# Structural-Variant-Calling-with-Pepper/pepper-thesis

Measured on AMD Instinct MI355X. Metric: pileup windows/sec (whole node) + Mbp/sec inferred, HG003 chr20 ONT R9, higher is better.
Workload: dtype f32

## Files before the change

### pepper_thesis_amd/csrc/rnn_bf16.hpp

```cpp
#pragma once
#include "pv_common.hpp"
#include "rnn_plan.hpp"

struct pv_gemm_desc {
    const unsigned char* A;
    const unsigned char* W;
    const float* bias;
    float* C;
    int64_t M;
    int N, K, splits, quads;
    const char* prof_name;
    int terms;
};
int pv_gemm_bf16x3_async(pv_ctx* ctx, const pv_gemm_desc& g, hipStream_t st);
int pv_gemm_bf16x3_prepare();
int pv_upload_split8(const float* w, size_t N, size_t K, unsigned char** d_split, std::vector<void*>& owned);
int pv_upload_split3(const float* w, size_t N, size_t K, unsigned char** d_planes, std::vector<void*>& owned);

struct pv_rec_desc {
    int cell;
    int enc;
    const float* G;
    const unsigned char* wp;
    const unsigned char* wx;
    const float* bias;
    const float* bias_hn;
    const void* x;
    int64_t x_row_bytes;
    int x_t0, xf, x_signed;
    int64_t B, Bp;
    int T;
    const float* h0;
    float* h_out;
    float* out_f32;
    unsigned char* out_tm;
    unsigned char* out_bm;
    int mt;
    const char* prof_name;
    int tr16;
    const unsigned char* dense_w;
    float* dense_part;
    int x6;
};
int pv_rec_bf16_async(pv_ctx* ctx, const pv_rec_desc& d, hipStream_t st);
int pv_rec_bf16_prepare();
int pv_pack_rec_bf16(const pv_rnn_dir* dirs, int cell, int kx, unsigned char** d_wp, unsigned char** d_wx, std::vector<void*>& owned,
                     int pieces = 2);
int pv_pack_gru16_bf16(const pv_rnn_dir* dirs, int kx, unsigned char** d_wp, unsigned char** d_wx, std::vector<void*>& owned);

struct pv_tail_desc {
    const float* part;
    int splits;
    int64_t part_rows;
    const float* b1;
    const unsigned char* wp;
    const float* b[4];
    const float* wo;
    const float* bo;
    float* probs;
    int64_t B;
    unsigned* epoch;
    const int* err;
};
int pv_tail_bf16_async(pv_ctx* ctx, const pv_tail_desc& d, hipStream_t st);
int pv_tail_bf16_prepare();
int pv_pack_tail_bf16(const float* const* w, unsigned char** d_wp, std::vector<void*>& owned);

struct pv_p2_bf16_weights {
    unsigned char* enc_wp = nullptr;
    unsigned char* enc_wx = nullptr;
    unsigned char* dec_wp = nullptr;
    float* enc_bias = nullptr;
    float* enc_bias_hn = nullptr;
    float* dec_bias_hn = nullptr;
    unsigned char* dec_wih_s = nullptr;
    unsigned char* dense_frag = nullptr;
    unsigned char* dense_frag16 = nullptr;
    unsigned char* enc16_wp = nullptr;
    unsigned char* enc16_wx = nullptr;
    unsigned char* dec16_wp = nullptr;
// ... 9 lines not shown
```

### pepper_thesis_amd/csrc/rnn_p1.hip

```cpp
#include "pv_common.hpp"
#include "rnn_bf16.hpp"
#include "rnn_f32.hpp"
#include "rnn_pack_host.hpp"

#include <algorithm>
#include <optional>

namespace {

constexpr int T_STEPS = PV_P1_T;
constexpr int F_IN = PV_P1_F;
constexpr int H = PV_P1_H;
constexpr int ROWS = PV_P1_ROWS;
constexpr int HEAD_N = PV_HEAD_N;
constexpr int HEAD_K = PV_HEAD_K;
constexpr int HEAD_MAX_SPLITS = PV_HEAD_MAX_SPLITS;

}

struct pv_rnn_p1 {
    float* enc_wp[2] = {nullptr, nullptr};
    float* dec_wp[2] = {nullptr, nullptr};
    float* enc_bias = nullptr; float* dec_bias = nullptr;
    float* enc_wps[2] = {nullptr, nullptr};
// ... 52 lines not shown
        pack_lstm(w->encoder, F_IN, 32, f ? 16 : 32, wp, bias);
        if ((rc = pv_dev_upload(wp, &m->enc_wp[f], m->owned))) return rc;
        if (!f && (rc = pv_dev_upload(bias, &m->enc_bias, m->owned))) return rc;
        pack_lstm(w->decoder, 2 * H, 2 * H, f ? 16 : 32, wp, bias);
        if ((rc = pv_dev_upload(wp, &m->dec_wp[f], m->owned))) return rc;
        if (!f && (rc = pv_dev_upload(bias, &m->dec_bias, m->owned))) return rc;
    }
    for (int f = 0; f < 2; f++) {
        pack_lstm_split(w->encoder, F_IN, 32, f ? 2 : 4, wp);
        if ((rc = pv_dev_upload(wp, &m->enc_wps[f], m->owned))) return rc;
        pack_lstm_split(w->decoder, 2 * H, 2 * H, f ? 2 : 4, wp);
        if ((rc = pv_dev_upload(wp, &m->dec_wps[f], m->owned))) return rc;
    }
    if ((rc = pv_dev_zeros(PV_LSTM_HX_BYTES, &m->sp_hx, m->owned)) || (rc = pv_dev_zeros(PV_LSTM_FLAGS_BYTES, &m->sp_flags, m->owned)) ||
        (rc = pv_dev_zeros(64, &m->sp_err, m->owned)) || (rc = pv_dev_zeros(64, &m->sp_epoch, m->owned)))
        return rc;
    pack_linear(w->linear_w[0], HEAD_K, 32, wp);
    if ((rc = pv_dev_upload(wp, &m->w1p, m->owned)) || (rc = pv_dev_upload(w->linear_b[0], HEAD_N, &m->b1, m->owned))) return rc;
    for (int i = 0; i < 4; i++) {
        for (int f = 0; f < 2; f++) {
            pack_linear(w->linear_w[i + 1], HEAD_N, f ? 16 : 32, wp);
            if ((rc = pv_dev_upload(wp, &m->wlp[f][i], m->owned))) return rc;
        }
        if ((rc = pv_dev_upload(w->linear_b[i + 1], HEAD_N, &m->bl[i], m->owned))) return rc;
    }
    if ((rc = pv_dev_upload(w->out_w, 3 * HEAD_N, &m->wo, m->owned)) || (rc = pv_dev_upload(w->out_b, 3, &m->bo, m->owned))) return rc;
    std::vector<float> wcat((size_t)2048 * 512), bcat(2048);
    for (int d = 0; d < 2; d++) {
        memcpy(&wcat[(size_t)d * 1024 * 512], w->decoder[d].w_ih, (size_t)1024 * 512 * sizeof(float));
        for (int n = 0; n < 1024; n++) bcat[d * 1024 + n] = w->decoder[d].b_ih[n] + w->decoder[d].b_hh[n];
    }
    if ((rc = pv_dev_upload(bcat, &m->dec_bias_cat, m->owned))) return rc;
    if (dtype == PV_DTYPE_F32) {
        if ((rc = pv_pack_rec_bf16(w->encoder, 4, F_IN, &m->enc_r6, nullptr, m->owned, 3))) return rc;
        if ((rc = pv_pack_rec_bf16(w->decoder, 4, 0, &m->dec_r6, nullptr, m->owned, 3))) return rc;
        if ((rc = pv_upload_split3(wcat.data(), 2048, 512, &m->dec_wih_p3, m->owned))) return rc;
        if ((rc = pv_upload_split3(w->linear_w[0], HEAD_N, HEAD_K, &m->w1_p3, m->owned))) return rc;
        if ((rc = pv_gemm_bf16x3_prepare()) || (rc = pv_rec_bf16_prepare())) return rc;
    }
    if (dtype == PV_DTYPE_BF16_INPUT_GEMM) {
        if ((rc = pv_upload_split8(wcat.data(), 2048, 512, &m->dec_wih_s, m->owned))) return rc;
        if ((rc = pv_upload_split8(w->linear_w[0], HEAD_N, HEAD_K, &m->w1_s, m->owned))) return rc;
        if ((rc = pv_pack_rec_bf16(w->encoder, 4, F_IN, &m->enc_rb, nullptr, m->owned))) return rc;
        if ((rc = pv_pack_rec_bf16(w->decoder, 4, 0, &m->dec_rb, nullptr, m->owned))) return rc;
        const float* tail_w[4] = {w->linear_w[1], w->linear_w[2], w->linear_w[3], w->linear_w[4]};
        if ((rc = pv_pack_tail_bf16(tail_w, &m->tail_wb, m->owned))) return rc;
        if ((rc = pv_gemm_bf16x3_prepare()) || (rc = pv_rec_bf16_prepare()) || (rc = pv_tail_bf16_prepare())) return rc;
    }
    if ((rc = pv_lstm_f32_prepare()) || (rc = pv_head_f32_prepare())) return rc;
    return PV_OK;
}

static int launch_tail(pv_ctx* ctx, const pv_p1_plan& pl, const float* part, int64_t part_rows, float* d_probs, int64_t B, hipStream_t st) {
    const pv_rnn_p1* m = ctx->p1;
    pv_head_tail_desc t = {};
    t.rows = pl.tail_rows; t.part = part; t.b1 = m->b1; t.splits = pl.splits; t.part_rows = part_rows;
    t.wo = m->wo; t.bo = m->bo; t.probs = d_probs; t.B = B; t.epoch = m->sp_epoch; t.err = m->sp_err;
    for (int i = 0; i < 4; i++) { t.wp[i] = m->wlp[pl.tail_rows == 16 ? 1 : 0][i]; t.b[i] = m->bl[i]; }
    int rc = pv_head_tail_async(ctx, t, st);
    if (rc) return rc;
    PV_HIP(hipGetLastError());
    return PV_OK;
}

struct P1Chain {
    int terms;
    const unsigned char *enc_rec, *dec_rec;
    const void *dec_wih, *w1;
// ... 166 lines not shown
```

### pepper_thesis_amd/csrc/rnn_pack_host.hpp

```cpp
#pragma once
#include <cstddef>
#include <cstdint>
#include <vector>

#include "../../include/pepper_hip.h"
#include "split3_host.hpp"

constexpr int PV_PACK_LSTM_H = 256;
constexpr int PV_PACK_GRU_H = 128;
constexpr int PV_PACK_NCLS = 5;
constexpr int PV_PACK_HEAD_N = 512;

static inline float pack_wval(const pv_rnn_dir& dir, int K, int KP, int HID, int n, int k) {
    if (k < KP) return k < K ? dir.w_ih[(size_t)n * K + k] : 0.0f;
    return dir.w_hh[(size_t)n * HID + (k - KP)];
}

static inline void pack_put_pieces(uint16_t* slot, int lane, int j, float v, int pieces = 2) {
    uint16_t p[3];
    split3_bits(v, p);
    for (int q = 0; q < pieces; q++) slot[512 * q + lane * 8 + j] = p[q];
}

static inline void split8_rows(const float* w, size_t N, size_t K, std::vector<uint16_t>& out) {
// ... 129 lines not shown

static inline void pack_rec_bf16(const pv_rnn_dir* dirs, int cell, int kx, int pieces, std::vector<uint16_t>& wp, std::vector<uint16_t>& wx) {
    const int NG = cell, HID = cell == 4 ? PV_PACK_LSTM_H : PV_PACK_GRU_H, NW = HID / 32, KS_H = HID / 16;
    const int KS_X = kx ? (cell == 4 ? 2 : 1) : 0;
    const bool xres = kx && cell == 3;
    const int nslot = (xres ? 0 : KS_X * NG) + KS_H * NG;
    const size_t SL = (size_t)pieces * 512;
    wp.assign((size_t)2 * NW * nslot * SL, 0);
    wx.assign(xres ? (size_t)2 * NW * NG * 1024 : 0, 0);
    for (int d = 0; d < 2; d++)
        for (int w = 0; w < NW; w++) {
            auto fill = [&](uint16_t* dst, bool xpart, int ks, int g) {
                for (int lane = 0; lane < 64; lane++)
                    for (int j = 0; j < 8; j++) {
                        const int n = g * HID + 32 * w + (lane & 31), k = 16 * ks + 8 * (lane >> 5) + j;
                        float v;
                        if (xpart) v = k < kx ? dirs[d].w_ih[(size_t)n * kx + k] : 0.0f;
                        else v = dirs[d].w_hh[(size_t)n * HID + k];
                        pack_put_pieces(dst, lane, j, v, pieces);
                    }
            };
            uint16_t* base = wp.data() + (size_t)(d * NW + w) * nslot * SL;
            int slot = 0;
            if (!xres)
                for (int ks = 0; ks < KS_X; ks++)
                    for (int g = 0; g < NG; g++) fill(base + (size_t)(slot++) * SL, true, ks, g);
            for (int ks = 0; ks < KS_H; ks++)
                for (int g = 0; g < NG; g++) fill(base + (size_t)(slot++) * SL, false, ks, g);
            if (xres)
                for (int g = 0; g < NG; g++) fill(wx.data() + ((size_t)(d * NW + w) * NG + g) * 1024, true, 0, g);
        }
}

static inline void pack_gru16_bf16(const pv_rnn_dir* dirs, int kx, std::vector<uint16_t>& wp, std::vector<uint16_t>& wx) {
    const int HID = PV_PACK_GRU_H, NW = 4;
    wp.assign((size_t)2 * NW * 24 * 1024, 0);
    wx.assign(kx ? (size_t)2 * NW * 6 * 1024 : 0, 0);
    for (int d = 0; d < 2; d++)
        for (int w = 0; w < NW; w++)
            for (int g = 0; g < 3; g++)
                for (int nt = 0; nt < 2; nt++) {
                    auto fill = [&](uint16_t* dst, bool xpart, int ks) {
                        for (int lane = 0; lane < 64; lane++)
                            for (int j = 0; j < 8; j++) {
                                const int n = g * HID + 32 * w + 16 * nt + (lane & 15), k = 32 * ks + 8 * (lane >> 4) + j;
                                const float v = xpart ? (k < kx ? dirs[d].w_ih[(size_t)n * kx + k] : 0.0f) : dirs[d].w_hh[(size_t)n * HID + k];
                                pack_put_pieces(dst, lane, j, v);
                            }
                    };
                    for (int ks = 0; ks < 4; ks++) fill(wp.data() + ((size_t)(d * NW + w) * 24 + (ks * 3 + g) * 2 + nt) * 1024, false, ks);
                    if (kx) fill(wx.data() + ((size_t)(d * NW + w) * 6 + g * 2 + nt) * 1024, true, 0);
                }
}

static inline void pack_tail_bf16(const float* const* w, std::vector<uint16_t>& wp) {
    constexpr int N = PV_PACK_HEAD_N, KS = N / 16;
    wp.assign((size_t)8 * 4 * KS * 2 * 1024, 0);
    for (int wv = 0; wv < 8; wv++)
        for (int l = 0; l < 4; l++)
            for (int ks = 0; ks < KS; ks++)
                for (int g = 0; g < 2; g++) {
                    uint16_t* dst = wp.data() + ((((size_t)wv * 4 + l) * KS + ks) * 2 + g) * 1024;
                    for (int lane = 0; lane < 64; lane++)
                        for (int j = 0; j < 8; j++) {
                            const int n = 64 * wv + 32 * g + (lane & 31), k = 16 * ks + 8 * (lane >> 5) + j;
                            pack_put_pieces(dst, lane, j, w[l][(size_t)n * N + k]);
// ... 32 lines not shown
```

### pepper_thesis_amd/csrc/rnn_rec_bf16.hip

```cpp
#include "rnn_bf16.hpp"
#include "mfma_tiles.hpp"
#include "rnn_math.hpp"
#include "rnn_p2_head.hpp"
#include "rnn_pack_host.hpp"

#include <algorithm>
#include <type_traits>
#include <cstdlib>

namespace {

using namespace pvdev;
typedef __bf16 bf16x8 __attribute__((ext_vector_type(8)));
typedef __bf16 bf16x4 __attribute__((ext_vector_type(4)));

__device__ __forceinline__ void split3_rest(float h, __bf16& x1, __bf16& x2) {
#pragma clang fp contract(off)
    const float r1 = h - (float)(__bf16)h;
    x1 = (__bf16)r1;
    x2 = (__bf16)(r1 - (float)x1);
}
__device__ __forceinline__ unsigned split8_off(unsigned k) { return (k >> 3) * 32u + (k & 7u) * 2u; }

template <int NG, bool ENC, int MT = 1, bool X6 = false> struct RecCfg {
    static constexpr int HID = NG == 4 ? 256 : 128;
    static constexpr int NW = HID / 32, NTHR = 64 * NW;
    static constexpr int KS_H = HID / 16;
    static constexpr int XK = ENC ? (NG == 4 ? 32 : 16) : 0;
    static constexpr int KS_X = XK / 16;
    static constexpr bool XRES = ENC && NG == 3;
    static constexpr bool WRES = NG == 3 && !(ENC && MT == 2);
    static constexpr int NSLOT = (XRES ? 0 : KS_X * NG) + KS_H * NG;
    static constexpr int D = ((NG == 3 && ENC) || (NG == 4 && MT == 2) || X6) ? 4 : 8;
    static constexpr int NA = NG + ((NG == 3 && ENC) ? 1 : 0);
    static constexpr int HS = HID * (X6 ? 8 : 4) + 16;
    static constexpr int H12 = X6 ? HID * 4 : 0;
    static constexpr int XS = XK * 2 + 16;
    static_assert(NSLOT % D == 0, "ring depth must divide the stream length");
};

struct RecArgs {
    const float* G;
    const unsigned char* wp;
    const unsigned char* wx;
    const float* bias;
    const float* bias_hn;
    const unsigned char* x;
    int64_t x_row_bytes;
    int x_t0, xf, x_signed;
    int64_t B, Bp;
    int T;
    const float* h0;
    float* h_out;
    float* out_f32;
    unsigned char* out_tm;
    unsigned char* out_bm;
    int n_tiles;
    const unsigned char* dw;
    float* dpart;
};

template <int NG, int MT, int NA, int D, int NTOT, int I0, int NKS, bool XP, bool X6 = false, int H12 = 0, typename Hook>
__device__ __forceinline__ void ring_bf16(f32x16 (&acc)[MT][NA], const unsigned char* __restrict__ At, int m_stride,
                                          __amdgpu_buffer_rsrc_t wr, f32x4 (&bq)[D][X6 ? 3 : 2], unsigned lane16, Hook&& hook) {
    constexpr int KSB = XP ? 32 : 64;
    constexpr int NP = X6 ? 3 : 2, SB = NP * 1024;
    bf16x8 ap[X6 && !XP ? 3 : 2][MT];
#pragma unroll
    for (int i = 0; i < NKS * NG; i++) {
        {
// ... 13 lines not shown
#pragma unroll
                    for (int j = 0; j < 8; j++) ap[0][m][j] = (__bf16)(j < 4 ? lo[j] : hi[j - 4]);
                } else {
                    ap[0][m] = *reinterpret_cast<const bf16x8*>(At + m * m_stride + ks * KSB);
                    if (!XP) ap[1][m] = *reinterpret_cast<const bf16x8*>(At + m * m_stride + ks * KSB + 16);
                }
            }
        }
        __builtin_amdgcn_sched_barrier(0);
        {
            const int ai = (XP && NG == 3 && g == 2) ? 3 : g;
            const int rs = (I0 + i) % D;
            const bf16x8 bh = __builtin_bit_cast(bf16x8, bq[rs][0]), bl = __builtin_bit_cast(bf16x8, bq[rs][1]);
#pragma unroll
            for (int m = 0; m < MT; m++) {
                if constexpr (X6) {
                    const bf16x8 b2 = __builtin_bit_cast(bf16x8, bq[rs][2]);
                    if constexpr (!XP) {
                        acc[m][ai] = __builtin_amdgcn_mfma_f32_32x32x16_bf16(ap[2][m], bh, acc[m][ai], 0, 0, 0);
                        acc[m][ai] = __builtin_amdgcn_mfma_f32_32x32x16_bf16(ap[1][m], bl, acc[m][ai], 0, 0, 0);
                    }
                    acc[m][ai] = __builtin_amdgcn_mfma_f32_32x32x16_bf16(ap[0][m], b2, acc[m][ai], 0, 0, 0);
                }
                acc[m][ai] = __builtin_amdgcn_mfma_f32_32x32x16_bf16(ap[0][m], bh, acc[m][ai], 0, 0, 0);
                acc[m][ai] = __builtin_amdgcn_mfma_f32_32x32x16_bf16(ap[0][m], bl, acc[m][ai], 0, 0, 0);
                if (!XP) acc[m][ai] = __builtin_amdgcn_mfma_f32_32x32x16_bf16(ap[1][m], bh, acc[m][ai], 0, 0, 0);
            }
        }
        hook(i);
        __builtin_amdgcn_sched_barrier(0);
    }
}

#ifndef PV_REC_ABL
#define PV_REC_ABL 0
#endif
#ifdef PV_REC_STAMPS
__device__ unsigned long long g_rec_stamps[8];
#define RSTAMP(i) { unsigned long long now_; asm volatile("s_memtime %0\n\ts_waitcnt lgkmcnt(0)" : "=s"(now_) :: "memory"); st_acc[i] += now_ - st_last; st_last = now_; }
#else
#define RSTAMP(i)
#endif

template <int NG, bool ENC, int MT, bool X6 = false>
__global__ __launch_bounds__(NG == 4 ? 512 : 256, 1) void k_rec_bf16(RecArgs a) {
    static_assert(!X6 || NG == 4, "split-6 form: LSTM only");
    typedef RecCfg<NG, ENC, MT, X6> C;
    constexpr int NP = X6 ? 3 : 2, SB = NP * 1024;
    constexpr int HID = C::HID, NW = C::NW, NTHR = C::NTHR, ROWS = 32 * MT, HS = C::HS, XS = C::XS, D = C::D, NA = C::NA;
    constexpr int NSLOT = C::NSLOT, NXS = C::XRES ? 0 : C::KS_X * NG;
    constexpr int NCOL = 2 * NG * HID;
    extern __shared__ __attribute__((aligned(16))) unsigned char sm[];
    unsigned char* hbuf = sm;
    unsigned char* xbuf = sm + 2 * ROWS * HS;
    const int tid = threadIdx.x, lane = tid & 63, wv = __builtin_amdgcn_readfirstlane(tid >> 6);
    const int xcd = blockIdx.x & 7;
    const int dir = xcd & 1;
    const int tile = (blockIdx.x >> 3) * 4 + (xcd >> 1);
    if (tile >= a.n_tiles) return;
    const int64_t b0 = (int64_t)tile * ROWS;
    const int unit = 32 * wv + (lane & 31), rg = lane >> 5;
    const int T = a.T;
    const __amdgpu_buffer_rsrc_t wr = make_rsrc(a.wp + (size_t)(dir * NW + wv) * NSLOT * SB);
    const unsigned lane16 = (unsigned)lane * 16u;
    f32x4 bq[C::WRES ? 1 : D][NP];
    bf16x8 wres[C::WRES ? NSLOT : 1][2];
    if constexpr (C::WRES) {
#pragma unroll
        for (int k = 0; k < NSLOT; k++) {
            wres[k][0] = __builtin_bit_cast(bf16x8, buf_load4(wr, lane16, (unsigned)(k * 2048)));
            wres[k][1] = __builtin_bit_cast(bf16x8, buf_load4(wr, lane16, (unsigned)(k * 2048 + 1024)));
        }
    } else {
#pragma unroll
        for (int k = 0; k < D - 1; k++)
#pragma unroll
            for (int p = 0; p < NP; p++) bq[k][p] = buf_load4(wr, lane16, (unsigned)(k * SB + p * 1024));
    }
    bf16x8 xw[C::XRES ? 3 : 1][2];
    if constexpr (C::XRES) {
        const __amdgpu_buffer_rsrc_t xr = make_rsrc(a.wx + (size_t)(dir * NW + wv) * 3 * 2048);
#pragma unroll
        for (int g = 0; g < 3; g++) {
            xw[g][0] = __builtin_bit_cast(bf16x8, buf_load4(xr, lane16, (unsigned)(g * 2048)));
            xw[g][1] = __builtin_bit_cast(bf16x8, buf_load4(xr, lane16, (unsigned)(g * 2048 + 1024)));
        }
    }
    float bs[NA];
    float b_hn = 0.0f;
    if constexpr (ENC) {
#pragma unroll
        for (int g = 0; g < NG; g++) bs[g] = a.bias[dir * NG * HID + g * HID + unit];
    }
    if constexpr (NG == 3) b_hn = a.bias_hn[dir * HID + unit];

    float st[MT][16];
    for (int i = tid; i < ROWS * HS / 16; i += NTHR) reinterpret_cast<u32x4*>(hbuf)[i] = u32x4{0u, 0u, 0u, 0u};
#pragma unroll
    for (int m = 0; m < MT; m++)
#pragma unroll
        for (int e = 0; e < 16; e++) st[m][e] = 0.0f;
    const unsigned hl = (unsigned)(4 * rg * HS) + (X6 ? (unsigned)unit * 4u : split8_off((unsigned)unit));
    const unsigned hl12 = (unsigned)(4 * rg * HS + C::H12) + split8_off((unsigned)unit);
    __syncthreads();
    if (NG == 3 && a.h0) {
#pragma unroll
        for (int m = 0; m < MT; m++)
#pragma unroll
            for (int e = 0; e < 16; e++) {
                const int row = 32 * m + 8 * (e >> 2) + (e & 3) + 4 * rg;
                const float h = a.h0[((b0 + row) * 2 + dir) * HID + unit];
                st[m][e] = h;
                const __bf16 hi = (__bf16)h;
                const __bf16 lo = (__bf16)(h - (float)hi);
                unsigned char* p = hbuf + (32 * m + 8 * (e >> 2) + (e & 3)) * HS + hl;
                *reinterpret_cast<__bf16*>(p) = hi;
                *reinterpret_cast<__bf16*>(p + 16) = lo;
            }
    }

    constexpr int FG = ENC ? C::XK / 4 : 1;
    const int xrow = tid / FG, xfg = tid % FG;
    const bool x_on = ENC && xrow < ROWS;
    const unsigned char* xsrc = nullptr;
    unsigned xv[4] = {0u, 0u, 0u, 0u};
    if constexpr (ENC) {
        int64_t r = b0 + xrow;
        if (r >= a.B) r = a.B - 1;
        xsrc = a.x + r * a.x_row_bytes + (int64_t)a.x_t0 * a.xf;
    }
    auto x_load = [&](int t) {
        if constexpr (ENC) {
            if (x_on) {
#pragma unroll
                for (int j = 0; j < 4; j++) {
                    const int f = 4 * xfg + j;
                    xv[j] = f < a.xf ? (unsigned)xsrc[(int64_t)t * a.xf + f] : 0u;
                }
            }
        }
    };
    auto x_store = [&](int slot) {
        if constexpr (ENC) {
            if (x_on) {
                bf16x4 v;
#pragma unroll
                for (int j = 0; j < 4; j++) {
                    const float f = a.x_signed ? (float)(int)(signed char)xv[j] : (float)xv[j];
                    v[j] = (__bf16)f;
                }
                *reinterpret_cast<bf16x4*>(xbuf + (slot * ROWS + xrow) * XS + xfg * 8) = v;
            }
        }
    };

    f32x16 acc[MT][NA];
    f32x4 gn[(NG == 3 && !ENC) ? MT : 1][4];
    const unsigned gl = (unsigned)((rg * NCOL + (lane & 31)) * 16);
    auto acc_init = [&](int t) {
        if constexpr (ENC) {
#pragma unroll
            for (int m = 0; m < MT; m++) {
#pragma unroll
                for (int g = 0; g < NG; g++)
#pragma unroll
                    for (int e = 0; e < 16; e++) acc[m][(NG == 3 && g == 2) ? 3 : g][e] = bs[g];
                if constexpr (NG == 3)
#pragma unroll
                    for (int e = 0; e < 16; e++) acc[m][2][e] = b_hn;
            }
        } else {
            const __amdgpu_buffer_rsrc_t gsr = make_rsrc(a.G + ((size_t)t * a.Bp + b0) * NCOL);
#pragma unroll
            for (int m = 0; m < MT; m++)
#pragma unroll
                for (int g = 0; g < NG; g++)
#pragma unroll
                    for (int q = 0; q < 4; q++) {
                        const f32x4 v = buf_load4_nt(gsr, gl, (unsigned)(((8 * m + 2 * q) * NCOL + dir * NG * HID + g * HID + 32 * wv) * 16));
                        if (NG == 3 && g == 2) {
                            gn[m][q] = v;
                        } else {
#pragma unroll
                            for (int j = 0; j < 4; j++) acc[m][g][4 * q + j] = v[j];
                        }
                    }
            if constexpr (NG == 3)
#pragma unroll
                for (int m = 0; m < MT; m++)
#pragma unroll
                    for (int e = 0; e < 16; e++) acc[m][2][e] = b_hn;
        }
    };

    x_load(dir ? T - 1 : 0);
    x_store(0);
    acc_init(dir ? T - 1 : 0);
    __syncthreads();

    const unsigned char* a_h = hbuf + (lane & 31) * HS + rg * 32;
    const unsigned char* a_x = xbuf + (lane & 31) * XS + rg * 16;
    const unsigned rowb_tm = 2u * HID * 4u;
    const unsigned rowb_bm = (unsigned)T * 2u * HID * 4u;
    const unsigned o_f_l = (unsigned)(4 * rg) * rowb_bm + (unsigned)unit * 4u;
    const __amdgpu_buffer_rsrc_t bmr = make_rsrc(a.out_bm + (size_t)b0 * rowb_bm);
    constexpr int CPR = HID / 4, NCP = ROWS * CPR / NTHR;
    const bool want_out = a.out_tm || a.out_bm;
    static_assert(NTHR % CPR == 0, "a piece is a whole number of rows");
    constexpr int RPP = NTHR / CPR;
    const unsigned cp_lds = (unsigned)((tid / CPR) * HS + (tid % CPR) * 16);
    const unsigned cp_tm = (unsigned)(tid / CPR) * rowb_tm + (unsigned)((tid % CPR) * 16);
    const unsigned cp_bm = (unsigned)(tid / CPR) * rowb_bm + (unsigned)((tid % CPR) * 16);
    u32x4 tile_v = {0u, 0u, 0u, 0u};
    auto tile_read = [&](int k, const unsigned char* tile) {
        tile_v = *reinterpret_cast<const u32x4*>(tile + k * RPP * HS + cp_lds);
    };
    auto tile_write = [&](int k, int tt) {
        if (a.out_tm) {
            const __amdgpu_buffer_rsrc_t tmr = make_rsrc(a.out_tm + ((size_t)tt * a.Bp + b0) * rowb_tm);
            __builtin_amdgcn_raw_buffer_store_b128(tile_v, tmr, cp_tm, (unsigned)(k * RPP) * rowb_tm + (unsigned)(dir * HID * 4), 2);
        }
        if (a.out_bm)
            __builtin_amdgcn_raw_buffer_store_b128(tile_v, bmr, cp_bm, (unsigned)(k * RPP) * rowb_bm + (unsigned)((tt * 2 + dir) * HID * 4), 2);
    };
    auto tile_out = [&](int tt, const unsigned char* tile) {
        if (!want_out) return;
#pragma unroll
        for (int k = 0; k < NCP; k++) { tile_read(k, tile); tile_write(k, tt); }
    };
    const __amdgpu_buffer_rsrc_t ofr = make_rsrc(reinterpret_cast<unsigned char*>(a.out_f32) + (size_t)b0 * rowb_bm);
    constexpr bool CAN_DENSE = NG == 3 && !ENC;
    const bool dense = CAN_DENSE && a.dpart != nullptr;
    bf16x8 dfr[CAN_DENSE ? 2 : 1][2];
    if constexpr (CAN_DENSE) {
// ... 7 lines not shown
        }
    }
    auto dense_out = [&](int tt, const unsigned char* tile) {
        if constexpr (CAN_DENSE) {
#pragma unroll
            for (int m = 0; m < MT; m++) {
                f32x16 ad;
#pragma unroll
                for (int e = 0; e < 16; e++) ad[e] = 0.0f;
#pragma unroll
                for (int k = 0; k < 2; k++) {
                    const unsigned char* At = tile + (lane & 31) * HS + rg * 32 + m * 32 * HS + (2 * wv + k) * 64;
                    const bf16x8 ah = *reinterpret_cast<const bf16x8*>(At), al = *reinterpret_cast<const bf16x8*>(At + 16);
                    ad = __builtin_amdgcn_mfma_f32_32x32x16_bf16(ah, dfr[k][0], ad, 0, 0, 0);
                    ad = __builtin_amdgcn_mfma_f32_32x32x16_bf16(ah, dfr[k][1], ad, 0, 0, 0);
                    ad = __builtin_amdgcn_mfma_f32_32x32x16_bf16(al, dfr[k][0], ad, 0, 0, 0);
                }
                if ((lane & 31) < 8) {
                    const size_t tile32 = (size_t)(b0 / 32) + m;
                    float* dst = a.dpart + ((((size_t)tt * (a.Bp / 32) + tile32) * 2 + dir) * 4 + wv) * 256 + (lane & 31) * 32 + 4 * rg;
#pragma unroll
                    for (int q = 0; q < 4; q++) {
                        f32x4 v;
#pragma unroll
                        for (int j = 0; j < 4; j++) v[j] = ad[4 * q + j];
                        *reinterpret_cast<f32x4*>(dst + 8 * q) = v;
                    }
                }
            }
        }
    };
    int cur = 0;
#ifdef PV_REC_STAMPS
    unsigned long long st_acc[5] = {0, 0, 0, 0, 0}, st_last;
    asm volatile("s_memtime %0\n\ts_waitcnt lgkmcnt(0)" : "=s"(st_last) :: "memory");
#endif
    for (int s = 0; s < T; s++) {
        const int t = dir ? (T - 1 - s) : s;
        const int tn = dir ? (T - 2 - s) : (s + 1);
        if (s + 1 < T) x_load(tn);
        const bool copy = want_out && s > 0;
        const int t_prev = dir ? t + 1 : t - 1;
        const unsigned char* tile_prev = hbuf + cur * ROWS * HS;
        constexpr int HSLOTS = C::KS_H * NG, HSTRIDE = HSLOTS / NCP;
        static_assert(HSTRIDE >= 2, "a piece needs two slots: read, then write");
        auto copy_hook = [&](int i) {
            if (copy) {
                if (i % HSTRIDE == 0 && i / HSTRIDE < NCP) tile_read(i / HSTRIDE, tile_prev);
                if (i % HSTRIDE == 1 && i / HSTRIDE < NCP) tile_write(i / HSTRIDE, t_prev);
            }
        };
        auto no_hook = [](int) {};
        if (NW == 8) { if (wv < 4) __builtin_amdgcn_s_setprio(3); else __builtin_amdgcn_s_setprio(0); }
        RSTAMP(0)
        if constexpr (C::XRES) {
            bf16x8 ax[MT];
#pragma unroll
            for (int m = 0; m < MT; m++) ax[m] = *reinterpret_cast<const bf16x8*>(a_x + ((s & 1) * ROWS + 32 * m) * XS);
#pragma unroll
            for (int g = 0; g < 3; g++)
#pragma unroll
                for (int m = 0; m < MT; m++) {
                    const int ai = g == 2 ? 3 : g;
                    acc[m][ai] = __builtin_amdgcn_mfma_f32_32x32x16_bf16(ax[m], xw[g][0], acc[m][ai], 0, 0, 0);
                    acc[m][ai] = __builtin_amdgcn_mfma_f32_32x32x16_bf16(ax[m], xw[g][1], acc[m][ai], 0, 0, 0);
                }
        } else if constexpr (ENC) {
            ring_bf16<NG, MT, NA, D, NSLOT, 0, C::KS_X, true, X6>(acc, a_x + (s & 1) * ROWS * XS, 32 * XS, wr, bq, lane16, no_hook);
        }
        if constexpr (C::WRES) {
            const unsigned char* At = a_h + cur * ROWS * HS;
#pragma unroll
            for (int ks = 0; ks < C::KS_H; ks++) {
                bf16x8 ah[MT], al[MT];
#pragma unroll
                for (int m = 0; m < MT; m++) {
                    ah[m] = *reinterpret_cast<const bf16x8*>(At + m * 32 * HS + ks * 64);
                    al[m] = *reinterpret_cast<const bf16x8*>(At + m * 32 * HS + ks * 64 + 16);
                }
#pragma unroll
                for (int g = 0; g < NG; g++)
#pragma unroll
                    for (int m = 0; m < MT; m++) {
                        acc[m][g] = __builtin_amdgcn_mfma_f32_32x32x16_bf16(ah[m], wres[ks * NG + g][0], acc[m][g], 0, 0, 0);
                        acc[m][g] = __builtin_amdgcn_mfma_f32_32x32x16_bf16(ah[m], wres[ks * NG + g][1], acc[m][g], 0, 0, 0);
                        acc[m][g] = __builtin_amdgcn_mfma_f32_32x32x16_bf16(al[m], wres[ks * NG + g][0], acc[m][g], 0, 0, 0);
                        if (m == MT - 1) copy_hook(ks * NG + g);
                    }
            }
        } else {
            ring_bf16<NG, MT, NA, D, NSLOT, NXS, C::KS_H, false, X6, C::H12>(acc, a_h + cur * ROWS * HS, 32 * HS, wr, bq, lane16, copy_hook);
        }
        if (dense && s > 0) dense_out(t_prev, tile_prev);
        if (NW == 8) { if (wv < 4) __builtin_amdgcn_s_setprio(2); else __builtin_amdgcn_s_setprio(1); }
        RSTAMP(1)
        unsigned char* hn = hbuf + (cur ^ 1) * ROWS * HS;
#pragma unroll
        for (int m = 0; m < MT; m++)
#pragma unroll
            for (int e = 0; e < 16; e++) {
                float h;
                if constexpr (NG == 4) {
#if PV_REC_ABL == 3
                    h = ((acc[m][0][e] + acc[m][1][e]) + acc[m][2][e]) + acc[m][3][e];
#else
                    const float ig = sigmoidf_(acc[m][0][e]);
                    const float fg = sigmoidf_(acc[m][1][e]);
                    const float gg = tanhf_(acc[m][2][e]);
                    const float og = sigmoidf_(acc[m][3][e]);
                    const float c = X6 ? __builtin_fmaf(fg, st[m][e], ig * gg) : fg * st[m][e] + ig * gg;
                    st[m][e] = c;
                    h = og * tanhf_(c);
#endif
                } else {
                    const float r = sigmoidf_(acc[m][0][e]);
                    const float z = sigmoidf_(acc[m][1][e]);
                    const float xn = ENC ? acc[m][NA - 1][e] : gn[ENC ? 0 : m][e >> 2][e & 3];
                    const float n = tanhf_(xn + r * acc[m][2][e]);
                    h = (1.0f - z) * n + z * st[m][e];
                    st[m][e] = h;
                }
                const int row = 32 * m + 8 * (e >> 2) + (e & 3);
#if PV_REC_ABL != 2
                if constexpr (X6) {
                    *reinterpret_cast<float*>(hn + row * HS + hl) = h;
                    {
                        __bf16 p1, p2;
                        split3_rest(h, p1, p2);
                        *reinterpret_cast<__bf16*>(hn + row * HS + hl12) = p1;
                        *reinterpret_cast<__bf16*>(hn + row * HS + hl12 + 16) = p2;
                    }
                } else {
                    const __bf16 hi = (__bf16)h;
                    const __bf16 lo = (__bf16)(h - (float)hi);
                    *reinterpret_cast<__bf16*>(hn + row * HS + hl) = hi;
                    *reinterpret_cast<__bf16*>(hn + row * HS + hl + 16) = lo;
                }
#endif
#if PV_REC_ABL == 1
                if (h == 123.456f)
#endif
                {
                if (a.out_f32) buf_store1_nt(h, ofr, o_f_l, (unsigned)row * rowb_bm + (unsigned)((t * 2 + dir) * HID * 4));
                }
            }
        RSTAMP(2)
        if (s + 1 < T) {
            acc_init(tn);
            x_store((s + 1) & 1);
        }
        cur ^= 1;
        RSTAMP(3)
        lds_barrier();
        RSTAMP(4)
    }
    tile_out(dir ? 0 : T - 1, hbuf + cur * ROWS * HS);
    if (dense) dense_out(dir ? 0 : T - 1, hbuf + cur * ROWS * HS);
#ifdef PV_REC_STAMPS
    if (blockIdx.x == 0 && lane == 0)
        for (int i = 0; i < 5; i++) atomicAdd(&g_rec_stamps[i], st_acc[i]);
#endif
    if (NG == 3 && a.h_out) {
#pragma unroll
        for (int m = 0; m < MT; m++)
#pragma unroll
            for (int e = 0; e < 16; e++) {
                const int row = 32 * m + 8 * (e >> 2) + (e & 3) + 4 * rg;
                a.h_out[((b0 + row) * 2 + dir) * HID + unit] = st[m][e];
            }
    }
}

constexpr int G16_HS = 128 * 4 + 16, G16_XS = 32 * 2 + 16;
template <bool ENC, int NTL>
__global__ __launch_bounds__(256, 1) void k_gru16_bf16(RecArgs a) {
    constexpr int HID = 128, NW = 4, ROWS = 16, HS = G16_HS, XS = G16_XS, NCOL = 6 * HID;
    __shared__ __attribute__((aligned(16))) unsigned char hbuf_all[NTL * 2 * ROWS * HS];
    __shared__ __attribute__((aligned(16))) unsigned char xbuf_all[ENC ? NTL * 2 * ROWS * XS : 16];
    const int tid = threadIdx.x, lane = tid & 63, wv = __builtin_amdgcn_readfirstlane(tid >> 6);
    const int xcd = blockIdx.x & 7, dir = xcd & 1;
    const int tile0 = ((blockIdx.x >> 3) * 4 + (xcd >> 1)) * NTL;
    if (tile0 >= a.n_tiles) return;
    const int lr = lane & 15, q = lane >> 4, T = a.T;
    const unsigned lane16 = (unsigned)lane * 16u;
    bf16x8 wres[24][2];
    {
        const __amdgpu_buffer_rsrc_t wr = make_rsrc(a.wp + (size_t)(dir * NW + wv) * 24 * 2048);
#pragma unroll
        for (int k = 0; k < 24; k++) {
            wres[k][0] = __builtin_bit_cast(bf16x8, buf_load4(wr, lane16, (unsigned)(k * 2048)));
            wres[k][1] = __builtin_bit_cast(bf16x8, buf_load4(wr, lane16, (unsigned)(k * 2048 + 1024)));
        }
    }
// ... 345 lines not shown
            s += __shfl_xor(s, 2, 64);
            s += __shfl_xor(s, 1, 64);
            if (sub == 0) logits[row][cls] = s + a.bo[cls];
        }
    }
    __syncthreads();
    if (tid < TL_ROWS) {
        const int64_t b = b0 + tid;
        if (b < a.B) {
            const float l0 = logits[tid][0], l1 = logits[tid][1], l2 = logits[tid][2];
            const float m = fmaxf(l0, fmaxf(l1, l2));
            const float e0 = expf(l0 - m), e1 = expf(l1 - m), e2 = expf(l2 - m);
            const float inv = 1.0f / (e0 + e1 + e2);
            const bool bad = a.err && a.err[0] != 0;
            const float nanv = __builtin_nanf("");
            a.probs[b * 3 + 0] = bad ? nanv : e0 * inv;
            a.probs[b * 3 + 1] = bad ? nanv : e1 * inv;
            a.probs[b * 3 + 2] = bad ? nanv : e2 * inv;
        }
    }
}
constexpr size_t LDS_TAIL_BF = (size_t)TL_ROWS * TL_HS;

}

int pv_pack_rec_bf16(const pv_rnn_dir* dirs, int cell, int kx, unsigned char** d_wp, unsigned char** d_wx, std::vector<void*>& owned,
                     int pieces) {
    PV_CHECK(pieces == 2 || (pieces == 3 && cell == 4), PV_ERR_INVALID, "three-piece fragments exist for the LSTM only");
    std::vector<uint16_t> wp, wx;
    pack_rec_bf16(dirs, cell, kx, pieces, wp, wx);
    if (d_wx) *d_wx = nullptr;
    int rc = pv_dev_upload(wp, d_wp, owned);
    return rc || wx.empty() ? rc : pv_dev_upload(wx, d_wx, owned);
}

int pv_pack_gru16_bf16(const pv_rnn_dir* dirs, int kx, unsigned char** d_wp, unsigned char** d_wx, std::vector<void*>& owned) {
    std::vector<uint16_t> wp, wx;
    pack_gru16_bf16(dirs, kx, wp, wx);
    if (d_wx) *d_wx = nullptr;
    int rc = pv_dev_upload(wp, d_wp, owned);
    return rc || wx.empty() ? rc : pv_dev_upload(wx, d_wx, owned);
}

int pv_pack_tail_bf16(const float* const* w, unsigned char** d_wp, std::vector<void*>& owned) {
    static_assert(TL_N == PV_PACK_HEAD_N, "pack_tail_bf16 packs 512 x 512 layers");
    std::vector<uint16_t> wp;
    pack_tail_bf16(w, wp);
    return pv_dev_upload(wp, d_wp, owned);
}

int pv_tail_bf16_prepare() {
    PV_HIP(hipFuncSetAttribute((const void*)k_tail_bf16, hipFuncAttributeMaxDynamicSharedMemorySize, (int)LDS_TAIL_BF));
    return PV_OK;
}

int pv_tail_bf16_async(pv_ctx* ctx, const pv_tail_desc& d, hipStream_t st) {
    PV_CHECK(d.part && d.wp && d.probs && d.B > 0 && d.splits >= 1, PV_ERR_INVALID, "bad tail launch");
    TailBfArgs a;
    a.part = d.part; a.splits = d.splits; a.part_rows = d.part_rows; a.b1 = d.b1; a.wp = d.wp;
    for (int i = 0; i < 4; i++) a.b[i] = d.b[i];
    a.wo = d.wo; a.bo = d.bo; a.probs = d.probs; a.B = d.B; a.epoch = d.epoch; a.err = d.err;
    pv_prof_scope ps(ctx, "k_tail_bf16", st);
    k_tail_bf16<<<(unsigned)((d.B + TL_ROWS - 1) / TL_ROWS), 512, LDS_TAIL_BF, st>>>(a);
    PV_HIP(hipGetLastError());
    return PV_OK;
}
// ... 183 lines not shown
        d.cell = 3; d.enc = 0; d.G = G; d.wp = w.dec_wp; d.bias_hn = w.dec_bias_hn; d.B = B; d.Bp = Bp; d.T = p2::WIN;
        d.h0 = state; d.h_out = state; d.mt = mt; d.prof_name = "k_rec_bf16_gru_dec";
        if (tr16) { d.tr16 = tr16; d.wp = w.dec16_wp; d.prof_name = "k_gru16_bf16_dec"; }
        float* lg_out = (d_logits && wi == nwin - 1) ? d_logits : nullptr;
        if (fold_dense) {
            d.dense_w = tr16 ? w.dense_frag16 : w.dense_frag; d.dense_part = dpart;
            if ((rc = pv_rec_bf16_async(ctx, d, st))) return rc;
            pv_prof_scope ps(ctx, "k_p2_combine", st);
            const int64_t nthr = (int64_t)p2::WIN * B;
            if (tr16) k_p2_combine<16><<<(unsigned)((nthr + 255) / 256), 256, 0, st>>>(dpart, Bp, B, w.dense_b, d_acc, seq, ws, lg_out);
            else k_p2_combine<32><<<(unsigned)((nthr + 255) / 256), 256, 0, st>>>(dpart, Bp, B, w.dense_b, d_acc, seq, ws, lg_out);
        } else {
            d.out_tm = dec;
            if ((rc = pv_rec_bf16_async(ctx, d, st))) return rc;
            pv_prof_scope ps(ctx, "k_p2_dense", st);
            const int64_t nthr = (int64_t)p2::WIN * B * 8;
            k_p2_dense<<<(unsigned)((nthr + 255) / 256), 256, 0, st>>>(dec, Bp, B, w.dense_w, w.dense_b, d_acc, seq, ws, lg_out);
        }
    }
    if (d_hidden_out) k_p2_state_out<<<(unsigned)((B * 2 * p2::HG + 255) / 256), 256, 0, st>>>(state, d_hidden_out, B);
    if (d_labels) k_p2_argmax<<<(unsigned)((B * seq + 255) / 256), 256, 0, st>>>(d_acc, B * seq, d_labels);
    PV_HIP(hipGetLastError());
    return PV_OK;
}

#ifdef PV_REC_STAMPS
extern "C" int pv_debug_rec_stamps(unsigned long long* out5) {
    unsigned long long z[8] = {0, 0, 0, 0, 0, 0, 0, 0};
    PV_HIP(hipDeviceSynchronize());
    PV_HIP(hipMemcpyFromSymbol(out5, HIP_SYMBOL(g_rec_stamps), 5 * sizeof(unsigned long long)));
    PV_HIP(hipMemcpyToSymbol(HIP_SYMBOL(g_rec_stamps), z, sizeof z));
    return PV_OK;
}
#endif
```

Baseline: 1.070 million.

## Use 16x16x32 MFMA tiles for split-6 LSTM recurrence with new weight packing

Switches the three-piece (split-6) f32-emulating LSTM recurrent kernel from 32x32x16 MFMA tiles to 16x16x32 tiles. It adds a matching host weight packer, new accumulator and bias layouts, and row/column remapping for the hidden-state writeback and output stores. The aim is better MFMA throughput or latency per recurrence step and a different register footprint on the serial time-step path. It also adds optional timing stamps behind a debug macro, and the old 32x32 path is kept behind a compile flag.

After: 1.105 million (median of 6 runs). 3.2% higher.

```diff
diff --git a/pepper_thesis_amd/csrc/rnn_bf16.hpp b/pepper_thesis_amd/csrc/rnn_bf16.hpp
--- a/pepper_thesis_amd/csrc/rnn_bf16.hpp
+++ b/pepper_thesis_amd/csrc/rnn_bf16.hpp
@@ -46,6 +46,7 @@
 int pv_rec_bf16_prepare();
 int pv_pack_rec_bf16(const pv_rnn_dir* dirs, int cell, int kx, unsigned char** d_wp, unsigned char** d_wx, std::vector<void*>& owned,
                      int pieces = 2);
+int pv_pack_rec_x6(const pv_rnn_dir* dirs, int kx, unsigned char** d_wp, std::vector<void*>& owned);
 int pv_pack_gru16_bf16(const pv_rnn_dir* dirs, int kx, unsigned char** d_wp, unsigned char** d_wx, std::vector<void*>& owned);
 
 struct pv_tail_desc {
diff --git a/pepper_thesis_amd/csrc/rnn_p1.hip b/pepper_thesis_amd/csrc/rnn_p1.hip
--- a/pepper_thesis_amd/csrc/rnn_p1.hip
+++ b/pepper_thesis_amd/csrc/rnn_p1.hip
@@ -108,8 +108,8 @@
     }
     if ((rc = pv_dev_upload(bcat, &m->dec_bias_cat, m->owned))) return rc;
     if (dtype == PV_DTYPE_F32) {
-        if ((rc = pv_pack_rec_bf16(w->encoder, 4, F_IN, &m->enc_r6, nullptr, m->owned, 3))) return rc;
-        if ((rc = pv_pack_rec_bf16(w->decoder, 4, 0, &m->dec_r6, nullptr, m->owned, 3))) return rc;
+        if ((rc = pv_pack_rec_x6(w->encoder, F_IN, &m->enc_r6, m->owned))) return rc;
+        if ((rc = pv_pack_rec_x6(w->decoder, 0, &m->dec_r6, m->owned))) return rc;
         if ((rc = pv_upload_split3(wcat.data(), 2048, 512, &m->dec_wih_p3, m->owned))) return rc;
         if ((rc = pv_upload_split3(w->linear_w[0], HEAD_N, HEAD_K, &m->w1_p3, m->owned))) return rc;
         if ((rc = pv_gemm_bf16x3_prepare()) || (rc = pv_rec_bf16_prepare())) return rc;
diff --git a/pepper_thesis_amd/csrc/rnn_pack_host.hpp b/pepper_thesis_amd/csrc/rnn_pack_host.hpp
--- a/pepper_thesis_amd/csrc/rnn_pack_host.hpp
+++ b/pepper_thesis_amd/csrc/rnn_pack_host.hpp
@@ -185,6 +185,28 @@
         }
 }
 
+static inline void pack_rec_x6_16(const pv_rnn_dir* dirs, int kx, std::vector<uint16_t>& wp) {
+    constexpr int HID = PV_PACK_LSTM_H, NW = HID / 32, KS_H = HID / 32, NG = 4;
+    const int nslot = (kx ? NG * 2 : 0) + KS_H * NG * 2;
+    constexpr size_t SL = 3 * 512;
+    wp.assign((size_t)2 * NW * nslot * SL, 0);
+    for (int d = 0; d < 2; d++)
+        for (int w = 0; w < NW; w++) {
+            uint16_t* dst = wp.data() + (size_t)(d * NW + w) * nslot * SL;
+            for (int ks = kx ? -1 : 0; ks < KS_H; ks++)
+                for (int g = 0; g < NG; g++)
+                    for (int c = 0; c < 2; c++, dst += SL)
+                        for (int lane = 0; lane < 64; lane++)
+                            for (int j = 0; j < 8; j++) {
+                                const int n = g * HID + 32 * w + 16 * c + (lane & 15), k = 8 * (lane >> 4) + j;
+                                float v;
+                                if (ks < 0) v = k < kx ? dirs[d].w_ih[(size_t)n * kx + k] : 0.0f;
+                                else v = dirs[d].w_hh[(size_t)n * HID + 32 * ks + k];
+                                pack_put_pieces(dst, lane, j, v, 3);
+                            }
+        }
+}
+
 static inline void pack_gru16_bf16(const pv_rnn_dir* dirs, int kx, std::vector<uint16_t>& wp, std::vector<uint16_t>& wx) {
     const int HID = PV_PACK_GRU_H, NW = 4;
     wp.assign((size_t)2 * NW * 24 * 1024, 0);
diff --git a/pepper_thesis_amd/csrc/rnn_rec_bf16.hip b/pepper_thesis_amd/csrc/rnn_rec_bf16.hip
--- a/pepper_thesis_amd/csrc/rnn_rec_bf16.hip
+++ b/pepper_thesis_amd/csrc/rnn_rec_bf16.hip
@@ -22,7 +22,14 @@
 }
 __device__ __forceinline__ unsigned split8_off(unsigned k) { return (k >> 3) * 32u + (k & 7u) * 2u; }
 
+#ifdef PV_REC_X6_MFMA32
+constexpr bool REC_X6_16 = false;
+#else
+constexpr bool REC_X6_16 = true;
+#endif
+
 template <int NG, bool ENC, int MT = 1, bool X6 = false> struct RecCfg {
+    static constexpr bool M16 = X6 && REC_X6_16;
     static constexpr int HID = NG == 4 ? 256 : 128;
     static constexpr int NW = HID / 32, NTHR = 64 * NW;
     static constexpr int KS_H = HID / 16;
@@ -35,7 +42,7 @@
     static constexpr int NA = NG + ((NG == 3 && ENC) ? 1 : 0);
     static constexpr int HS = HID * (X6 ? 8 : 4) + 16;
     static constexpr int H12 = X6 ? HID * 4 : 0;
-    static constexpr int XS = XK * 2 + 16;
+    static constexpr int XS = M16 ? 96 : XK * 2 + 16;
     static_assert(NSLOT % D == 0, "ring depth must divide the stream length");
 };
 
@@ -115,11 +122,62 @@
     }
 }
 
+template <int D, int NTOT, int I0, int NKS, bool XP, int H12, typename Hook>
+__device__ __forceinline__ void ring_x6_16(f32x4 (&acc)[2][4][2], const unsigned char* __restrict__ At, int m_stride,
+                                           __amdgpu_buffer_rsrc_t wr, f32x4 (&bq)[D][3], unsigned lane16, Hook&& hook) {
+    constexpr int KSB = XP ? 64 : 128;
+    bf16x8 ap[XP ? 1 : 3][2];
+#pragma unroll
+    for (int i = 0; i < NKS * 8; i++) {
+        {
+            const int sv = (I0 + i + D - 1) % NTOT, rs = (I0 + i + D - 1) % D;
+#pragma unroll
+            for (int p = 0; p < 3; p++) bq[rs][p] = buf_load4(wr, lane16, (unsigned)(sv * 3072 + p * 1024));
+        }
+        const int ks = i / 8, g = (i / 2) % 4, c = i % 2;
+        if (i % 8 == 0) {
+#pragma unroll
+            for (int m = 0; m < 2; m++) {
+                if constexpr (!XP) {
+                    const f32x4 lo = *reinterpret_cast<const f32x4*>(At + m * m_stride + ks * KSB);
+                    const f32x4 hi = *reinterpret_cast<const f32x4*>(At + m * m_stride + ks * KSB + 16);
+                    ap[1][m] = *reinterpret_cast<const bf16x8*>(At + m * m_stride + ks * KSB + H12);
+                    ap[2][m] = *reinterpret_cast<const bf16x8*>(At + m * m_stride + ks * KSB + H12 + 16);
+#pragma unroll
+                    for (int j = 0; j < 8; j++) ap[0][m][j] = (__bf16)(j < 4 ? lo[j] : hi[j - 4]);
+                } else {
+                    ap[0][m] = *reinterpret_cast<const bf16x8*>(At + m * m_stride + ks * KSB);
+                }
+            }
+        }
+        __builtin_amdgcn_sched_barrier(0);
+        {
+            const int rs = (I0 + i) % D;
+            const bf16x8 b0 = __builtin_bit_cast(bf16x8, bq[rs][0]), b1 = __builtin_bit_cast(bf16x8, bq[rs][1]);
+            const bf16x8 b2 = __builtin_bit_cast(bf16x8, bq[rs][2]);
+#define PV_X6_TERM(AP, BP)          \
+    _Pragma("unroll") for (int m = 0; m < 2; m++) acc[m][g][c] = __builtin_amdgcn_mfma_f32_16x16x32_bf16(ap[AP][m], BP, acc[m][g][c], 0, 0, 0);
+            if constexpr (!XP) {
+                PV_X6_TERM(2, b0)
+                PV_X6_TERM(1, b1)
+            }
+            PV_X6_TERM(0, b2)
+            PV_X6_TERM(0, b0)
+            PV_X6_TERM(0, b1)
+            if constexpr (!XP) { PV_X6_TERM(1, b0) }
+#undef PV_X6_TERM
+        }
+        hook(i);
+        __builtin_amdgcn_sched_barrier(0);
+    }
+}
+
 #ifndef PV_REC_ABL
 #define PV_REC_ABL 0
 #endif
 #ifdef PV_REC_STAMPS
 __device__ unsigned long long g_rec_stamps[8];
+#define RSTAMP_REAL(v) asm volatile("s_memrealtime %0\n\ts_waitcnt lgkmcnt(0)" : "=s"(v) :: "memory");
 #define RSTAMP(i) { unsigned long long now_; asm volatile("s_memtime %0\n\ts_waitcnt lgkmcnt(0)" : "=s"(now_) :: "memory"); st_acc[i] += now_ - st_last; st_last = now_; }
 #else
 #define RSTAMP(i)
@@ -130,6 +188,7 @@
     static_assert(!X6 || NG == 4, "split-6 form: LSTM only");
     typedef RecCfg<NG, ENC, MT, X6> C;
     constexpr int NP = X6 ? 3 : 2, SB = NP * 1024;
+    constexpr bool M16 = C::M16;
     constexpr int HID = C::HID, NW = C::NW, NTHR = C::NTHR, ROWS = 32 * MT, HS = C::HS, XS = C::XS, D = C::D, NA = C::NA;
     constexpr int NSLOT = C::NSLOT, NXS = C::XRES ? 0 : C::KS_X * NG;
     constexpr int NCOL = 2 * NG * HID;
@@ -142,7 +201,7 @@
     const int tile = (blockIdx.x >> 3) * 4 + (xcd >> 1);
     if (tile >= a.n_tiles) return;
     const int64_t b0 = (int64_t)tile * ROWS;
-    const int unit = 32 * wv + (lane & 31), rg = lane >> 5;
+    const int unit = 32 * wv + (M16 ? (lane & 15) : (lane & 31)), rg = M16 ? lane >> 4 : lane >> 5;
     const int T = a.T;
     const __amdgpu_buffer_rsrc_t wr = make_rsrc(a.wp + (size_t)(dir * NW + wv) * NSLOT * SB);
     const unsigned lane16 = (unsigned)lane * 16u;
@@ -170,8 +229,14 @@
         }
     }
     float bs[NA];
+    float bs16[M16 && ENC ? 4 : 1][2];
     float b_hn = 0.0f;
-    if constexpr (ENC) {
+    if constexpr (M16 && ENC) {
+#pragma unroll
+        for (int g = 0; g < 4; g++)
+#pragma unroll
+            for (int c = 0; c < 2; c++) bs16[g][c] = a.bias[dir * NG * HID + g * HID + unit + 16 * c];
+    } else if constexpr (ENC) {
 #pragma unroll
         for (int g = 0; g < NG; g++) bs[g] = a.bias[dir * NG * HID + g * HID + unit];
     }
@@ -237,11 +302,23 @@
         }
     };
 
-    f32x16 acc[MT][NA];
+    f32x16 acc[M16 ? 1 : MT][M16 ? 1 : NA];
+    f32x4 acc16[M16 ? 2 : 1][4][2];
     f32x4 gn[(NG == 3 && !ENC) ? MT : 1][4];
-    const unsigned gl = (unsigned)((rg * NCOL + (lane & 31)) * 16);
+    const unsigned gl = (unsigned)((rg * NCOL + (M16 ? (lane & 15) : (lane & 31))) * 16);
     auto acc_init = [&](int t) {
-        if constexpr (ENC) {
+        if constexpr (M16) {
+            const __amdgpu_buffer_rsrc_t gsr = make_rsrc(ENC ? nullptr : a.G + ((size_t)t * a.Bp + b0) * NCOL);
+#pragma unroll
+            for (int mi = 0; mi < 2; mi++)
+#pragma unroll
+                for (int g = 0; g < 4; g++)
+#pragma unroll
+                    for (int c = 0; c < 2; c++) {
+                        if constexpr (ENC) acc16[mi][g][c] = f32x4{bs16[g][c], bs16[g][c], bs16[g][c], bs16[g][c]};
+                        else acc16[mi][g][c] = buf_load4_nt(gsr, gl, (unsigned)((4 * mi * NCOL + dir * NG * HID + g * HID + 32 * wv + 16 * c) * 16));
+                    }
+        } else if constexpr (ENC) {
 #pragma unroll
             for (int m = 0; m < MT; m++) {
 #pragma unroll
@@ -281,8 +358,8 @@
     acc_init(dir ? T - 1 : 0);
     __syncthreads();
 
-    const unsigned char* a_h = hbuf + (lane & 31) * HS + rg * 32;
-    const unsigned char* a_x = xbuf + (lane & 31) * XS + rg * 16;
+    const unsigned char* a_h = hbuf + (lane & (M16 ? 15 : 31)) * HS + rg * 32;
+    const unsigned char* a_x = xbuf + (lane & (M16 ? 15 : 31)) * XS + rg * 16;
     const unsigned rowb_tm = 2u * HID * 4u;
     const unsigned rowb_bm = (unsigned)T * 2u * HID * 4u;
     const unsigned o_f_l = (unsigned)(4 * rg) * rowb_bm + (unsigned)unit * 4u;
@@ -356,8 +433,10 @@
     };
     int cur = 0;
 #ifdef PV_REC_STAMPS
-    unsigned long long st_acc[5] = {0, 0, 0, 0, 0}, st_last;
+    unsigned long long st_acc[5] = {0, 0, 0, 0, 0}, st_last, st_real0, st_real1;
+    RSTAMP_REAL(st_real0)
     asm volatile("s_memtime %0\n\ts_waitcnt lgkmcnt(0)" : "=s"(st_last) :: "memory");
+    const unsigned long long st_first = st_last;
 #endif
     for (int s = 0; s < T; s++) {
         const int t = dir ? (T - 1 - s) : s;
@@ -389,6 +468,8 @@
                     acc[m][ai] = __builtin_amdgcn_mfma_f32_32x32x16_bf16(ax[m], xw[g][0], acc[m][ai], 0, 0, 0);
                     acc[m][ai] = __builtin_amdgcn_mfma_f32_32x32x16_bf16(ax[m], xw[g][1], acc[m][ai], 0, 0, 0);
                 }
+        } else if constexpr (M16 && ENC) {
+            ring_x6_16<D, NSLOT, 0, 1, true, 0>(acc16, a_x + (s & 1) * ROWS * XS, 16 * XS, wr, bq, lane16, no_hook);
         } else if constexpr (ENC) {
             ring_bf16<NG, MT, NA, D, NSLOT, 0, C::KS_X, true, X6>(acc, a_x + (s & 1) * ROWS * XS, 32 * XS, wr, bq, lane16, no_hook);
         }
@@ -412,6 +493,8 @@
                         if (m == MT - 1) copy_hook(ks * NG + g);
                     }
             }
+        } else if constexpr (M16) {
+            ring_x6_16<D, NSLOT, NXS, HID / 32, false, C::H12>(acc16, a_h + cur * ROWS * HS, 16 * HS, wr, bq, lane16, copy_hook);
         } else {
             ring_bf16<NG, MT, NA, D, NSLOT, NXS, C::KS_H, false, X6, C::H12>(acc, a_h + cur * ROWS * HS, 32 * HS, wr, bq, lane16, copy_hook);
         }
@@ -419,6 +502,10 @@
         if (NW == 8) { if (wv < 4) __builtin_amdgcn_s_setprio(2); else __builtin_amdgcn_s_setprio(1); }
         RSTAMP(1)
         unsigned char* hn = hbuf + (cur ^ 1) * ROWS * HS;
+        auto gsum = [&](int m, int g, int e) -> float {
+            if constexpr (M16) return acc16[e >> 3][g][(e >> 2) & 1][e & 3];
+            else return acc[m][g][e];
+        };
 #pragma unroll
         for (int m = 0; m < MT; m++)
 #pragma unroll
@@ -426,12 +513,12 @@
                 float h;
                 if constexpr (NG == 4) {
 #if PV_REC_ABL == 3
-                    h = ((acc[m][0][e] + acc[m][1][e]) + acc[m][2][e]) + acc[m][3][e];
+                    h = ((gsum(m, 0, e) + gsum(m, 1, e)) + gsum(m, 2, e)) + gsum(m, 3, e);
 #else
-                    const float ig = sigmoidf_(acc[m][0][e]);
-                    const float fg = sigmoidf_(acc[m][1][e]);
-                    const float gg = tanhf_(acc[m][2][e]);
-                    const float og = sigmoidf_(acc[m][3][e]);
+                    const float ig = sigmoidf_(gsum(m, 0, e));
+                    const float fg = sigmoidf_(gsum(m, 1, e));
+                    const float gg = tanhf_(gsum(m, 2, e));
+                    const float og = sigmoidf_(gsum(m, 3, e));
                     const float c = X6 ? __builtin_fmaf(fg, st[m][e], ig * gg) : fg * st[m][e] + ig * gg;
                     st[m][e] = c;
                     h = og * tanhf_(c);
@@ -444,15 +531,16 @@
                     h = (1.0f - z) * n + z * st[m][e];
                     st[m][e] = h;
                 }
-                const int row = 32 * m + 8 * (e >> 2) + (e & 3);
+                const int row = M16 ? 16 * (e >> 3) + (e & 3) : 32 * m + 8 * (e >> 2) + (e & 3);
+                const int cb = M16 ? 64 * ((e >> 2) & 1) : 0;
 #if PV_REC_ABL != 2
                 if constexpr (X6) {
-                    *reinterpret_cast<float*>(hn + row * HS + hl) = h;
+                    *reinterpret_cast<float*>(hn + row * HS + cb + hl) = h;
                     {
                         __bf16 p1, p2;
                         split3_rest(h, p1, p2);
-                        *reinterpret_cast<__bf16*>(hn + row * HS + hl12) = p1;
-                        *reinterpret_cast<__bf16*>(hn + row * HS + hl12 + 16) = p2;
+                        *reinterpret_cast<__bf16*>(hn + row * HS + cb + hl12) = p1;
+                        *reinterpret_cast<__bf16*>(hn + row * HS + cb + hl12 + 16) = p2;
                     }
                 } else {
                     const __bf16 hi = (__bf16)h;
@@ -465,7 +553,7 @@
                 if (h == 123.456f)
 #endif
                 {
-                if (a.out_f32) buf_store1_nt(h, ofr, o_f_l, (unsigned)row * rowb_bm + (unsigned)((t * 2 + dir) * HID * 4));
+                if (a.out_f32) buf_store1_nt(h, ofr, o_f_l, (unsigned)row * rowb_bm + (unsigned)((t * 2 + dir) * HID * 4 + cb));
                 }
             }
         RSTAMP(2)
@@ -478,11 +566,17 @@
         lds_barrier();
         RSTAMP(4)
     }
+#ifdef PV_REC_STAMPS
+    RSTAMP_REAL(st_real1)
+#endif
     tile_out(dir ? 0 : T - 1, hbuf + cur * ROWS * HS);
     if (dense) dense_out(dir ? 0 : T - 1, hbuf + cur * ROWS * HS);
 #ifdef PV_REC_STAMPS
-    if (blockIdx.x == 0 && lane == 0)
+    if (blockIdx.x == 0 && lane == 0) {
         for (int i = 0; i < 5; i++) atomicAdd(&g_rec_stamps[i], st_acc[i]);
+        atomicAdd(&g_rec_stamps[5], st_last - st_first);
+        atomicAdd(&g_rec_stamps[6], st_real1 - st_real0);
+    }
 #endif
     if (NG == 3 && a.h_out) {
 #pragma unroll
@@ -894,6 +988,13 @@
     if (d_wx) *d_wx = nullptr;
     int rc = pv_dev_upload(wp, d_wp, owned);
     return rc || wx.empty() ? rc : pv_dev_upload(wx, d_wx, owned);
+}
+
+int pv_pack_rec_x6(const pv_rnn_dir* dirs, int kx, unsigned char** d_wp, std::vector<void*>& owned) {
+    std::vector<uint16_t> wp, wx;
+    if (REC_X6_16) pack_rec_x6_16(dirs, kx, wp);
+    else pack_rec_bf16(dirs, 4, kx, 3, wp, wx);
+    return pv_dev_upload(wp, d_wp, owned);
 }
 
 int pv_pack_gru16_bf16(const pv_rnn_dir* dirs, int kx, unsigned char** d_wp, unsigned char** d_wx, std::vector<void*>& owned) {
@@ -1143,4 +1244,9 @@
     PV_HIP(hipMemcpyToSymbol(HIP_SYMBOL(g_rec_stamps), z, sizeof z));
     return PV_OK;
 }
+extern "C" int pv_debug_rec_clock(unsigned long long* out2) {
+    PV_HIP(hipDeviceSynchronize());
+    PV_HIP(hipMemcpyFromSymbol(out2, HIP_SYMBOL(g_rec_stamps), 2 * sizeof(unsigned long long), 5 * sizeof(unsigned long long)));
+    return PV_OK;
+}
 #endif
```
